# oleg-savchenko/jax_nbody_emulator_with_dj

Measured on AMD Instinct MI355X. Metric: voxels/sec (disp+vel) on 512^3 box, ndiv=4, higher is better.
Workload: dtype f32-equivalent: f16x3 split MFMA (3 f16 MFMAs per product, f32 accumulate)

## Files before the change

jax_nbody_emulator_with_dj_amd/csrc/nbe_engine.cpp:

```cpp

#include "../../include/nbe.h"
#include "nbe_kernels.h"

#include <sched.h>

#include <cmath>
#include <cstdarg>
#include <cstdio>
#include <cstdlib>
#include <cstring>
#include <algorithm>
#include <atomic>
#include <chrono>
#include <condition_variable>
#include <deque>
#include <map>
#include <memory>
#include <mutex>
#include <string>
#include <thread>
#include <vector>

using namespace nbe;

// ... 1261 lines not shown
                                  "up_r2", "conv_r2", "up_r1", "conv_r1", "up_r0", "conv_r00", "conv_r01"};

static int pack_wino(nbe_ctx* c) {
    c->wino_ok = false;
    if (!((c->prec == PREC_F16X3 && (c->vel ? c->gauge_active : true)) || (c->prec == PREC_F16 && c->vel && c->gauge_active))) return 0;
    if (!c->wino_flag) HIPCHK(hipMalloc((void**)&c->wino_flag, 4));
    HIPCHK(hipMemsetAsync(c->wino_flag, 0, 4, c->stream));
    for (auto& kv : c->layers) {
        Layer& L = kv.second;
        if (L.pw.ww && L.kind == 0 && (L.g6 || !c->vel)) launch_pack_h3w(L.wn, L.cout, L.cin, L.pw.cin_pad, L.pw.ctiles, L.pw.ww, c->wino_flag, c->stream, c->prec);
        if (L.pw.ww && L.kind == 1 && (c->vel ? (L.b_sub && c->fuse) : c->novel_fuse)) {
            launch_pack_h3w_skip(L.wn, L.cout, L.cin, L.pw, L.pw.ww, c->wino_flag, c->stream);
            if (c->vel) launch_pack_h3w_skip(c->prec == PREC_F16 ? L.dwn_f : L.dwn, L.cout, L.cin, L.pw, L.pw.ww + L.pw.floats, c->wino_flag, c->stream);
        }
    }
    int bad = 0;
    HIPCHK(hipMemcpyAsync(&bad, c->wino_flag, 4, hipMemcpyDeviceToHost, c->stream));
    HIPCHK(hipStreamSynchronize(c->stream));
    c->wino_ok = bad == 0;
    if (!c->vel) c->fuse = c->novel_fuse && c->wino_ok;
    if (c->prec == PREC_F16) c->fuse = c->fuse && c->wino_ok;
    return 0;
}

static int wire_novel(nbe_ctx* c) {
    c->novel_fuse = false;
    if (c->vel || c->prec != PREC_F16X3) return 0;
    for (const char* b : kBlocks) {
        if (!strncmp(b, "down_", 5) || !strncmp(b, "up_", 3)) continue;
        auto i1 = c->layers.find(std::string(b) + "/conv_1"), is = c->layers.find(std::string(b) + "/skip");
        if (i1 == c->layers.end() || is == c->layers.end()) return fail("internal: block %s", b);
        Layer &L1 = i1->second, &Ls = is->second;
        if (!L1.pw.ww || !Ls.pw.ww || 2 * (Ls.pw.cin_pad / 16) > 16 || L1.pw.ctiles != Ls.pw.ctiles) return 0;
    }
    for (const char* b : kBlocks) {
        if (!strncmp(b, "down_", 5) || !strncmp(b, "up_", 3)) continue;
        Layer &L1 = c->layers[std::string(b) + "/conv_1"], &Ls = c->layers[std::string(b) + "/skip"];
        L1.fskip = &Ls;
        const int nb = L1.pw.ctiles * 32 * L1.pw.ni;
        HIPCHK(hipMalloc((void**)&L1.bias_f, nb * 4));
    }
    c->novel_fuse = true;
    return 0;
}

static int wire_gauge(nbe_ctx* c) {
    const int m = c->mid;
    for (auto& kv : c->layers) {
        Layer& L = kv.second;
        const size_t na = (size_t)roundup(L.cin, 16) + 64, nb = (size_t)L.pw.ctiles * 32 * L.pw.ni + 64;
        HIPCHK(hipMalloc((void**)&L.alpha, na * 4)); HIPCHK(hipMemset(L.alpha, 0, na * 4));
        HIPCHK(hipMalloc((void**)&L.beta, nb * 4)); HIPCHK(hipMemset(L.beta, 0, nb * 4));
    }
    if (!c->gauge_flag) HIPCHK(hipMalloc((void**)&c->gauge_flag, 4));
    auto lay = [&](const char* b, const char* l) -> Layer* {
        auto it = c->layers.find(std::string(b) + "/" + l);
        return it == c->layers.end() ? nullptr : &it->second;
    };
    struct Rule { const char* pb; const char* pl; const char* consumer; int off; };
    const Rule rules[] = {
        {"conv_l00", "conv_1", "conv_l01", 0}, {"conv_l01", "conv_1", "conv_r00", 0}, {"down_l0", "conv_0", "conv_l1", 0},
        {"conv_l1", "conv_1", "conv_r1", 0},   {"down_l1", "conv_0", "conv_l2", 0},   {"conv_l2", "conv_1", "conv_r2", 0},
        {"down_l2", "conv_0", "conv_c", 0},    {"up_r2", "conv_0", "conv_r2", m},     {"up_r1", "conv_0", "conv_r1", m},
        {"up_r0", "conv_0", "conv_r00", m},    {"conv_r00", "conv_1", "conv_r01", 0},
    };
    for (const Rule& r : rules) {
        Layer *P = lay(r.pb, r.pl), *C = lay(r.consumer, "conv_0");
        if (!P || !C || r.off + P->cout > C->cin) return fail("internal: gauge wiring %s/%s -> %s", r.pb, r.pl, r.consumer);
        P->gout = C->alpha + r.off;
    }
    for (const char* b : kBlocks) {
        if (!strncmp(b, "down_", 5) || !strncmp(b, "up_", 3)) continue;
        Layer *L0 = lay(b, "conv_0"), *L1 = lay(b, "conv_1"), *Ls = lay(b, "skip");
        L0->gout = L1->alpha;
        L1->g6 = true;
        if (strcmp(b, "conv_l00")) { L0->g6 = true; Ls->a_in = L0->alpha; }
        if (c->prec == PREC_F16X3 && (!L1->pwn.w || Ls->pwn.dw) &&
            3 * (L1->pw.cin_pad / 16) + Ls->pw.cin_pad / 16 <= NBE_MAX_GROUPS) {
            L1->fskip = Ls; Ls->b_sub = L1->beta;
            const int nb = L1->pw.ctiles * 32 * L1->pw.ni;
            HIPCHK(hipMalloc((void**)&L1->bias_f, nb * 4));
        }
        if (c->prec == PREC_F16 && L1->pw.ww && Ls->pw.ww && Ls->dwn_f && L1->pw.ctiles == Ls->pw.ctiles &&
            2 * (Ls->pw.cin_pad / 32) <= 16) {
            L1->fskip = Ls; Ls->b_sub = L1->beta;
            const int nb = L1->pw.ctiles * 32 * L1->pw.ni;
            HIPCHK(hipMalloc((void**)&L1->bias_f, nb * 4));
        }
    }
    for (auto& kv : c->layers)
        if (kv.second.g6 && 3 * (kv.second.pw.cin_pad / 16) > NBE_MAX_GROUPS) { c->gauge = false; return 0; }
    lay("down_l0", "conv_0")->a_in = lay("conv_r00", "conv_0")->alpha;
    lay("down_l1", "conv_0")->a_in = lay("conv_r1", "conv_0")->alpha;
    lay("down_l2", "conv_0")->a_in = lay("conv_r2", "conv_0")->alpha;
    c->gauge = true;
    return 0;
}

static int wire_gauge_premod(nbe_ctx* c, const nbe_layer_desc* descs, int n) {
    std::map<std::string, std::vector<double>> al, be;
    std::map<std::string, const nbe_layer_desc*> by_name;
    for (int i = 0; i < n; ++i) by_name[std::string(descs[i].block) + "/" + descs[i].layer] = &descs[i];
    for (const char* b : kBlocks) {
        if (!strncmp(b, "down_", 5) || !strncmp(b, "up_", 3)) continue;
        for (const char* l : {"conv_0", "conv_1"}) {
            if (!strcmp(b, "conv_l00") && !strcmp(l, "conv_0")) continue;
            const std::string key = std::string(b) + "/" + l;
            const nbe_layer_desc& d = *by_name[key];
            const int co = d.cout, ci = d.cin, k3 = d.k * d.k * d.k;
            std::vector<double> a(ci, 0.0), bt(co, 0.0);
            double dmax = 0.0;
            for (size_t e = 0; e < (size_t)co * ci * k3; ++e) dmax = std::max(dmax, (double)std::fabs(d.dweight[e]));
            for (int iter = 0; iter < 200; ++iter) {
                double change = 0.0;
                for (int i = 0; i < ci; ++i) {
                    double num = 0.0, den = 0.0;
                    for (int o = 0; o < co; ++o)
                        for (int k = 0; k < k3; ++k) {
                            const double w = d.weight[((size_t)o * ci + i) * k3 + k], dw = d.dweight[((size_t)o * ci + i) * k3 + k];
                            num += w * (dw - w * bt[o]); den += w * w;
                        }
                    const double v = den > 0 ? num / den : 0.0;
                    change = std::max(change, std::fabs(v - a[i])); a[i] = v;
                }
                for (int o = 0; o < co; ++o) {
                    double num = 0.0, den = 0.0;
                    for (int i = 0; i < ci; ++i)
                        for (int k = 0; k < k3; ++k) {
                            const double w = d.weight[((size_t)o * ci + i) * k3 + k], dw = d.dweight[((size_t)o * ci + i) * k3 + k];
                            num += w * (dw - w * a[i]); den += w * w;
                        }
                    const double v = den > 0 ? num / den : 0.0;
                    change = std::max(change, std::fabs(v - bt[o])); bt[o] = v;
                }
                if (change < 1e-13) break;
            }
            double res = 0.0;
            for (int o = 0; o < co; ++o)
                for (int i = 0; i < ci; ++i)
                    for (int k = 0; k < k3; ++k) {
                        const size_t e = ((size_t)o * ci + i) * k3 + k;
                        res = std::max(res, std::fabs((double)d.dweight[e] - (double)d.weight[e] * (a[i] + bt[o])));
                    }
            if (!(res <= 2e-6 * dmax + 1e-30)) return 0;
            const double amin = *std::min_element(a.begin(), a.end()), amax = *std::max_element(a.begin(), a.end());
            const double mid = 0.5 * (amin + amax);
            for (double& v : a) v -= mid;
            for (double& v : bt) v += mid;
            if (amax - mid > 64.0) return 0;
            al[key] = a; be[key] = bt;
        }
    }
    if (wire_gauge(c)) return 1;
    if (!c->gauge) return 0;
    for (auto& kv : c->layers) {
        Layer& L = kv.second;
        auto ia = al.find(kv.first);
        if (ia != al.end()) {
            std::vector<float> fa(ia->second.begin(), ia->second.end()), fb(be[kv.first].begin(), be[kv.first].end());
            HIPCHK(hipMemcpy(L.alpha, fa.data(), fa.size() * 4, hipMemcpyHostToDevice));
            HIPCHK(hipMemcpy(L.beta, fb.data(), fb.size() * 4, hipMemcpyHostToDevice));
        }
    }
    auto fold = [&](const char* b, const char* l, const char* reader, int off) -> int {
        const std::string key = std::string(b) + "/" + l;
        const nbe_layer_desc& d = *by_name[key];
        Layer& L = c->layers[key];
// ... 1325 lines not shown
```

jax_nbody_emulator_with_dj_amd/csrc/nbe_kernels_wino.h:

```cpp

#ifndef NBE_EPI_MAX
#define NBE_EPI_MAX 1
#endif
#ifndef NBE_WINO_ZROW
#define NBE_WINO_ZROW 1
#endif
#ifndef NBE_WINO_ITEMREG
#define NBE_WINO_ITEMREG 1
#endif
#ifndef NBE_WINO_LOU
#define NBE_WINO_LOU (NBE_XF_F32 ? 0 : 1)
#endif
constexpr int NBE_MAX_WSTAGES = 32;
constexpr int NBE_MAX_WSKIP = 16;
constexpr float WINO_WSCALE = 16384.0f;
constexpr float WINO_WSCALE_F16 = 256.0f;

struct WinoSrc { const char* xa; const char* xb; long dxd; const char* w; long psb; float sb; int pad_; };

struct WinoKArgs {
    int H, W, Dv, Hv, Wv, Ho, Wo;
    int nchunk, cout_groups, flags, ntiles, tny, tnx;
    int zblock;
    float* y; float* dy; long out_pstride; int out_g0;
    const float* bias; const float* gout; const float* beta;
    const float* r; const float* dr; long res_pstride;
    float inv_scale;
    int nskip;
    long dws_delta;
    WinoSrc st[NBE_MAX_WSTAGES + NBE_MAX_WSKIP];
};

template <bool SKIP, bool NOVEL, bool F16 = false>
__global__ __launch_bounds__(512, 2) void conv_h3w_kernel(WinoKArgs a) {
    static_assert(!(F16 && NOVEL), "the float16 form has no displacement-only variant");
    typedef HGGeom<false> G;
    constexpr int NW = 8, CT = 64, TAPU = G::TAPU, WGU = G::WG, XBASE = G::XBASE, MT = 4, NT = 2, NTILE = 8;
    constexpr int ZROW = G::LDS_UNITS;
    f32x4* lds = lds_h3;
    const half8* L8 = (const half8*)lds_h3;
    half8* L8w = (half8*)lds_h3;
    const int tid = threadIdx.x;
    const int lane = tid & 63;
    const int wave = __builtin_amdgcn_readfirstlane(tid >> 6);
    const int c = lane & 15, q = lane >> 4, kh = q & 1, ks = q >> 1;

    const int nct = (a.cout_groups + 7) / 8;
    const int vt = xcd_tile(blockIdx.x, a.ntiles * nct);
    const int tile = vt / nct, ct = vt - tile * nct;
    const int npair = a.Dv >> 1;
    int zp, ty, tx;
    {
        const int zb = a.zblock;
        const int full = (npair / zb) * zb;
        const int per_blk = zb * a.tny * a.tnx;
        if (tile < (npair / zb) * per_blk) {
            const int blk = tile / per_blk, r = tile - blk * per_blk;
            const int zi = r % zb, tyx = r / zb;
            zp = blk * zb + zi; ty = tyx / a.tnx; tx = tyx - ty * a.tnx;
        } else {
            const int r = tile - (npair / zb) * per_blk, rem = npair - full;
            const int zi = r % rem, tyx = r / rem;
            zp = full + zi; ty = tyx / a.tnx; tx = tyx - ty * a.tnx;
        }
    }
    const int y0 = ty * (NOVEL ? 2 * HP_ROWS : HP_ROWS), x0 = tx * HP_COLS, z0 = 2 * zp;
    const int nst = 4 * a.nchunk;

    const long to = (((long)z0 * a.H + y0) * a.W + x0) * 16;
    const long wcm = (long)ct * nst * WGU * 16, wcs = (long)ct * a.nskip * TAPU * 16;

    struct Nxt { const char *xa, *xb, *w0; long dxd, psb; float sb; } nx;
    auto set_next = [&](int s) {
        const WinoSrc e = a.st[s];
        nx.xa = e.xa + to; nx.xb = e.xb + to; nx.dxd = e.dxd; nx.psb = e.psb; nx.w0 = e.w + (SKIP && s >= nst ? wcs : wcm); nx.sb = e.sb;
    };
    unsigned lane16 = (unsigned)lane << 4;
    asm volatile("" : "+v"(lane16));
    auto dma_w = [&](int buf, int t) {
        const int n = wave + NW * t;
        unsigned l16 = (unsigned)lane;
        if (NBE_WINO_ZROW && !F16) l16 = lane16;
        else asm volatile("v_lshlrev_b32 %0, 4, %0" : "+v"(l16));
        if (n < G::NWI) dma16s(nx.w0 + (long)n * 1024, l16, lds + buf * WGU + n * 64);
    };
    auto dma_raw = [&](int buf) {
        unsigned l16 = (unsigned)lane;
        asm volatile("v_lshlrev_b32 %0, 4, %0" : "+v"(l16));
        dma16s(nx.w0 + (wave < 4 ? 0 : a.dws_delta) + (long)(wave & 3) * 1024, l16, lds + buf * WGU + wave * 64);
#pragma unroll
        for (int t = 0; t < 6; ++t) {
            const int tensor = t / 3, n = wave + NW * (t % 3), pl = n / 6, k = n - 6 * pl;
            const int u = k * 64 + lane;
            const int uu = u < HP_PL ? u : HP_PL - 1;
            const int row = (uu * 241) >> 13, col = uu - row * HP_RS;
            if (u < HP_PL)
                dma16s(nx.xa + (tensor ? nx.dxd : 0) + (long)pl * nx.psb, (unsigned)(row * a.W + col) * 16u,
                       lds + XBASE + buf * HQ_XB + tensor * HQ_XT + pl * HQ_PP + k * 64);
        }
    };
    constexpr bool ITEMREG = NBE_WINO_ITEMREG && !F16;
    int it_uu[3] = {0, 0, 0};
    unsigned it_go[3] = {0u, 0u, 0u};
    if (ITEMREG) {
#pragma unroll
        for (int j = 0; j < 3; ++j) {
            const int u = ((wave + NW * j) % 6) * 64 + lane;
            it_uu[j] = u < HP_PL ? u : HP_PL - 1;
            const int row = (it_uu[j] * 241) >> 13, col = it_uu[j] - row * HP_RS;
            it_go[j] = (unsigned)(row * a.W + col) * 16u;
        }
#pragma unroll
        for (int j = 0; j < 3; ++j) asm volatile("" : "+v"(it_uu[j]), "+v"(it_go[j]));
    }
    auto item_unit = [&](int j, bool& valid) {
        if (ITEMREG) {
            valid = lane < HP_PL - ((wave + NW * j) % 6) * 64;
            return it_uu[j];
        }
        int l = lane;
        asm volatile("" : "+v"(l));
        const int u = ((wave + NW * j) % 6) * 64 + l;
        valid = u < HP_PL;
        return valid ? u : HP_PL - 1;
    };
    auto item_goff_j = [&](int j) {
        if (ITEMREG) return it_go[j];
        bool v;
        const int uu = item_unit(j, v);
        const int row = (uu * 241) >> 13, col = uu - row * HP_RS;
        return (unsigned)(row * a.W + col) * 16u;
    };
    typedef unsigned int u32x4 __attribute__((ext_vector_type(4)));
    struct Stg { half8 ah, al, bh, bl; float sb; };
    auto st_load = [&](int j, Stg& g) {
        const int n = wave + NW * j;
        const long po = ((n / 12) ? nx.dxd : 0) + (long)(((n % 12) / 6) * 2) * nx.psb;
        const char* pa = nx.xa + po;
        const char* pb = nx.xb + po;
        const unsigned go = item_goff_j(j);
        const __amdgpu_buffer_rsrc_t ra = __builtin_amdgcn_make_buffer_rsrc((void*)pa, 0, 0xffffffffu, 0x00027000);
        const __amdgpu_buffer_rsrc_t rb = __builtin_amdgcn_make_buffer_rsrc((void*)pb, 0, 0xffffffffu, 0x00027000);
        const unsigned pso = (unsigned)nx.psb;
        auto ld = [&](half8& d, __amdgpu_buffer_rsrc_t r, unsigned so) {
            const u32x4 v = __builtin_amdgcn_raw_buffer_load_b128(r, go, so, 0);
            d = __builtin_bit_cast(half8, v);
        };
        ld(g.ah, ra, 0); ld(g.al, ra, pso); ld(g.bh, rb, 0); ld(g.bl, rb, pso);
        g.sb = nx.sb;
    };
#if NBE_XF_F32
    struct Xf { u32x4 HI, LO; float t0, t1; unsigned h; };
    auto xf_step = [&](const Stg& g, Xf& x, int k) {
        const int r = k >> 2, m = k & 3;
        const unsigned AH = __builtin_bit_cast(u32x4, g.ah)[r], AL = __builtin_bit_cast(u32x4, g.al)[r];
        const unsigned BH = __builtin_bit_cast(u32x4, g.bh)[r], BL = __builtin_bit_cast(u32x4, g.bl)[r];
        const float inv = H3_INV, sinv = g.sb * H3_INV, sb = g.sb, k2048 = H3_SCALE;
        if (m == 0) {
            asm("v_fma_mix_f32 %0, %1, %2, %3 op_sel:[0,0,0] op_sel_hi:[1,0,1]" : "=v"(x.t0) : "v"(AL), "s"(inv), "v"(AH));
            asm("v_fma_mix_f32 %0, %1, %2, %0 op_sel:[0,0,0] op_sel_hi:[1,0,0]" : "+v"(x.t0) : "v"(BL), "s"(sinv));
            asm("v_fma_mix_f32 %0, %1, %2, %0 op_sel:[0,0,0] op_sel_hi:[1,0,0]" : "+v"(x.t0) : "v"(BH), "s"(sb));
        } else if (m == 1) {
            asm("v_fma_mix_f32 %0, %1, %2, %3 op_sel:[1,0,1] op_sel_hi:[1,0,1]" : "=v"(x.t1) : "v"(AL), "s"(inv), "v"(AH));
            asm("v_fma_mix_f32 %0, %1, %2, %0 op_sel:[1,0,0] op_sel_hi:[1,0,0]" : "+v"(x.t1) : "v"(BL), "s"(sinv));
            asm("v_fma_mix_f32 %0, %1, %2, %0 op_sel:[1,0,0] op_sel_hi:[1,0,0]" : "+v"(x.t1) : "v"(BH), "s"(sb));
        } else if (m == 2) {
            asm("v_cvt_pk_f16_f32 %0, %1, %2" : "=v"(x.h) : "v"(x.t0), "v"(x.t1));
            asm("v_fma_mix_f32 %0, %1, -1.0, %0 op_sel:[0,0,0] op_sel_hi:[1,0,0]" : "+v"(x.t0) : "v"(x.h));
            asm("v_fma_mix_f32 %0, %1, -1.0, %0 op_sel:[1,0,0] op_sel_hi:[1,0,0]" : "+v"(x.t1) : "v"(x.h));
        } else {
            unsigned l;
            asm("v_fma_mixlo_f16 %0, %1, %2, 0 op_sel_hi:[0,0,0]" : "=v"(l) : "v"(x.t0), "s"(k2048));
            asm("v_fma_mixhi_f16 %0, %1, %2, 0 op_sel_hi:[0,0,0]" : "+v"(l) : "v"(x.t1), "s"(k2048));
            x.HI[r] = x.h; x.LO[r] = l;
        }
    };
#else
    struct Xf { u32x4 HI, LO; unsigned s, bb, e1, e2, l1; };
    auto xf_step = [&](const Stg& g, Xf& x, int k) {
        const int r = k >> 2, m = k & 3;
        const unsigned AH = __builtin_bit_cast(u32x4, g.ah)[r], AL = __builtin_bit_cast(u32x4, g.al)[r];
// ... 130 lines not shown
        NBE_SB; MM8h(DY, wh, dxh, slot0 < 0 ? -1 : slot0 + 4, nb, px, false, hooked, [&](int t) { hook(8 + t); }); NBE_SB;
        after3();
        mid();
#if NBE_WINO_LOU
        NBE_SB; MM8(DY, wh, dxl, -1, nb, px); NBE_SB;
#else
        NBE_SB; MM8(DY, wp, dxl, -1, nb, px); NBE_SB;
#endif
        preXl(); preW();
        NBE_SB; MM8(Y, wl, xh, -1, nb, px); NBE_SB;
        preXh();
        NBE_SB; MM8(DY, wl, dxh, -1, nb, px); NBE_SB;
    };

    constexpr int SH4 = HP_RS + 1, SH5 = HP_RS + 2, SH7 = 2 * HP_RS + 1;
    auto stage = [&](f32x4 (&Y)[NTILE], f32x4 (&DY)[NTILE], int s, auto nxt) {
        constexpr int NXT = decltype(nxt)::value;
        constexpr bool px = NXT == 1;
        const bool pre = px && s + 1 != 2 * a.nchunk;
        if (NXT) set_next(s + 1);
        int par = s & 1;
        asm volatile("" : "+s"(par));
        int nb = 1 - par;
        asm volatile("" : "+s"(nb));
        const int wb = par * WGU, xb = XBASE + par * HQ_XB;
        const int wbn = nb * WGU, xbn = XBASE + nb * HQ_XB;
        Stg g;
        Xf xf;
        auto hk = [&](int k) { xf_step(g, xf, k); };
        auto none = [] {};
        if (NXT == 2) dma_raw(nb);
        if (px) st_load(0, g);
        pair(Y, DY, 0, nb, px, wb, xb + bP1,
             [&] { LB(xl, xb + 2 + bP32 + HQ_PP); }, [&] { LA(wh, wb + 2 * TAPU + aP); }, [&] { LB(xh, xb + 2 + bP32); },
             none, false, nohook, none);
        half8 a1[MT], a2[MT], b1x[NT], b1d[NT];
        const int aS = wb + 4 * TAPU + (2 * kh + (F16 ? ks : 0)) * CT + c;
        const int bS = xb + (2 * kh + ks) * HQ_PP + rowp * HP_RS + c + SH4;
        pair(Y, DY, -1, nb, px, wb + 2 * TAPU, xb + 2 + bP32,
             [&] { LB(b1x, bS); }, [&] { LA(a1, aS); }, [&] { LB(b1d, bS + HQ_XT); }, none,
             px, hk, [&] { if (px) { st_write(0, nb, xf); st_load(1, g); } });
        const half8 zero = {0, 0, 0, 0, 0, 0, 0, 0};
        if (F16) {
            NBE_SB; MM8(Y, a1, b1x, -1, 0, false); NBE_SB;
            LB(xl, xb + SH5 + bP32 + HQ_PP); LB(xh, xb + SH5 + bP32); LA(wh, wb + 5 * TAPU + aP);
            NBE_SB; MM8(DY, a1, b1d, -1, 0, false); NBE_SB;
        } else {
#if NBE_WINO_LOU
        NBE_SB; MM8(Y, a1, b1x, -1, 0, false); NBE_SB;
#else
        {
            const _Float16 m1 = ks ? kInv : (_Float16)1.0f;
#pragma unroll
            for (int mt = 0; mt < MT; ++mt) a1[mt] = a1[mt] * m1;
        }
        NBE_SB; MM8(Y, a1, b1x, -1, 0, false, true); NBE_SB;
#endif
#if NBE_WINO_ZROW
        LA(a2, ks ? ZROW + c : aS + CT);
#else
        LA(a2, aS + CT);
#endif
        LB(xl, xb + SH5 + bP32 + HQ_PP);
        NBE_SB; MM8(DY, a1, b1d, -1, 0, false); NBE_SB;
        LB(xh, xb + SH5 + bP32); LA(wh, wb + 5 * TAPU + aP);
#if NBE_WINO_ZROW
        NBE_SB; MM8(Y, a2, b1x, -1, 0, false); NBE_SB;
#else
#pragma unroll
        for (int mt = 0; mt < MT; ++mt) a2[mt] = ks ? zero : a2[mt];
        NBE_SB; MM8(Y, a2, b1x, -1, 0, false, true); NBE_SB;
#endif
        MM8(DY, a2, b1d, -1, 0, false); NBE_SB;
        }
        pair(Y, DY, -1, nb, px, wb + 5 * TAPU, xb + SH5 + bP32,
             [&] { LB(xl, xb + SH7 + bP1 + HQ_PP); }, [&] { LA(wh, wb + 7 * TAPU + aP); }, [&] { LB(xh, xb + SH7 + bP1); },
             none, px, hk, [&] { if (px) { st_write(1, nb, xf); st_load(2, g); } });
        pair(Y, DY, -1, nb, px, wb + 7 * TAPU, xb + SH7 + bP1,
             [&] { if (pre) LB(xl, xbn + bP1 + HQ_PP); }, [&] { if (pre) LA(wh, wbn + aP); }, [&] { if (pre) LB(xh, xbn + bP1); },
             [&] { asm volatile("s_waitcnt vmcnt(0) lgkmcnt(0)\n\ts_barrier" ::: "memory"); },
             px, hk, [&] { if (px) st_write(2, nb, xf); });
    };

    auto raw_stage = [&](f32x4 (&Y)[NTILE], f32x4 (&DY)[NTILE], int s, bool px) {
        if (px) set_next(s + 1);
        int par = s & 1;
        asm volatile("" : "+s"(par));
        int nb = 1 - par;
        asm volatile("" : "+s"(nb));
        const int wb = par * WGU, xb = XBASE + par * HQ_XB;
        if (px) dma_raw(nb);
        half8 a1[MT], a2[MT], d1[MT], d2[MT], bx[NT], bd[NT];
        const half8 zero = {0, 0, 0, 0, 0, 0, 0, 0};
        const _Float16 m1 = ks ? kInv : (_Float16)1.0f;
        const int aS = wb + (2 * kh) * CT + c;
        const int bS = xb + (2 * kh + ks) * HQ_PP + rowp * HP_RS + c + SH4;
        if (F16) {
            const int aF = wb + (2 * kh + ks) * CT + c;
            LA(a1, aF); LB(bx, bS); LB(bd, bS + HQ_XT); LA(d1, aF + TAPU);
            NBE_SB; MM8(Y, a1, bx, -1, 0, false); NBE_SB;
            MM8(DY, a1, bd, -1, 0, false); NBE_SB;
            MM8(DY, d1, bx, -1, 0, false); NBE_SB;
            asm volatile("s_waitcnt vmcnt(0) lgkmcnt(0)\n\ts_barrier" ::: "memory");
            return;
        }
        LA(a1, aS); LB(bx, bS); LA(a2, aS + CT); LB(bd, bS + HQ_XT);
#pragma unroll
        for (int mt = 0; mt < MT; ++mt) a1[mt] = a1[mt] * m1;
        NBE_SB; MM8(Y, a1, bx, -1, 0, false, true); NBE_SB;
        if (!NOVEL) LA(d1, aS + TAPU);
#pragma unroll
        for (int mt = 0; mt < MT; ++mt) a2[mt] = ks ? zero : a2[mt];
        NBE_SB; MM8(Y, a2, bx, -1, 0, false, true); NBE_SB;
        if (!NOVEL) LA(d2, aS + TAPU + CT);
        if (NOVEL || !(a.flags & F_SKIP_NODX)) {
            NBE_SB; MM8(DY, a1, bd, -1, 0, false); NBE_SB;
            MM8(DY, a2, bd, -1, 0, false); NBE_SB;
        }
        if (!NOVEL) {
#pragma unroll
            for (int mt = 0; mt < MT; ++mt) { d1[mt] = d1[mt] * m1; d2[mt] = ks ? zero : d2[mt]; }
            NBE_SB; MM8(DY, d1, bx, -1, 0, false, true); NBE_SB;
            MM8(DY, d2, bx, -1, 0, false, true); NBE_SB;
        }
        asm volatile("s_waitcnt vmcnt(0) lgkmcnt(0)\n\ts_barrier" ::: "memory");
    };

    {
        if (NBE_WINO_ZROW && !F16 && tid < 64) L8w[ZROW + tid] = half8{0, 0, 0, 0, 0, 0, 0, 0};
        set_next(0);
#pragma unroll
        for (int k = 0; k < G::NWS; ++k) dma_w(0, k);
        {
            Stg g0, g1, g2;
            st_load(0, g0); st_load(1, g1); st_load(2, g2);
            st_store(0, 0, g0); st_store(1, 0, g1); st_store(2, 0, g2);
        }
        asm volatile("s_waitcnt vmcnt(0) lgkmcnt(0)" ::: "memory");
        __syncthreads();
        LA(wh, aP); LB(xl, XBASE + bP1 + HQ_PP); LB(xh, XBASE + bP1);
    }

    auto butterfly = [&] {
            asm volatile("s_nop 15\n\ts_nop 15" ::: "memory");
#pragma unroll
            for (int t = 0; t < NTILE; ++t) {
                f32x4 p, m;
#pragma unroll
                for (int e = 0; e < 4; ++e) { p[e] = acc_read(YA[t][e]); m[e] = acc_read(YB[t][e]); }
                YA[t] = p + m; YB[t] = p - m;
                asm volatile("" : "+a"(YA[t]), "+a"(YB[t]));
                __builtin_amdgcn_sched_barrier(0);
#pragma unroll
                for (int e = 0; e < 4; ++e) { p[e] = acc_read(DA[t][e]); m[e] = acc_read(DB[t][e]); }
                DA[t] = p + m; DB[t] = p - m;
                asm volatile("" : "+a"(DA[t]), "+a"(DB[t]));
                __builtin_amdgcn_sched_barrier(0);
            }
            asm volatile("s_nop 7" ::: "memory");
            LA(wh, aP); LB(xl, XBASE + bP1 + HQ_PP); LB(xh, XBASE + bP1);
    };
    const int npairs = 2 * a.nchunk;
    for (int s2 = 0; s2 + 1 < npairs; ++s2) {
        if (s2 == a.nchunk) butterfly();
        stage(YA, DA, 2 * s2, std::integral_constant<int, 1>());
        stage(YB, DB, 2 * s2 + 1, std::integral_constant<int, 1>());
    }
    if (npairs - 1 == a.nchunk) butterfly();
    stage(YA, DA, 2 * npairs - 2, std::integral_constant<int, 1>());
    stage(YB, DB, 2 * npairs - 1, std::integral_constant<int, SKIP ? 2 : 0>());
    if (SKIP) {
        for (int sc = 0; sc < a.nskip; ++sc) {
            raw_stage(YA, DA, nst + 2 * sc, true);
            raw_stage(YB, DB, nst + 2 * sc + 1, sc + 1 < a.nskip);
        }
    }
#undef NBE_SB
#undef SNAKE
    asm volatile("s_nop 15\n\ts_nop 15" ::: "memory");

    const bool act = a.flags & F_ACT, gauge = !NOVEL && a.gout != nullptr;
    f32x4 bv[MT], be[MT], gv[MT];
    int unit[MT];
    bool uok[MT];
#pragma unroll
    for (int mt = 0; mt < MT; ++mt) {
        unit[mt] = ct * (CT / 8) + 2 * mt + ks;
        uok[mt] = unit[mt] < a.cout_groups;
        if (!uok[mt]) unit[mt] = a.cout_groups - 1;
        bv[mt] = *(const f32x4*)(a.bias + unit[mt] * 8 + 4 * kh);
        be[mt] = f32x4{0.f, 0.f, 0.f, 0.f};
        if (!NOVEL) be[mt] = *(const f32x4*)(a.beta + unit[mt] * 8 + 4 * kh);
        gv[mt] = f32x4{0.f, 0.f, 0.f, 0.f};
        if (!NOVEL && gauge) gv[mt] = *(const f32x4*)(a.gout + unit[mt] * 8 + 4 * kh);
    }
#pragma unroll
    for (int mt = 0; mt < MT; ++mt) asm volatile("" : "+v"(bv[mt]), "+v"(be[mt]), "+v"(gv[mt]));
    long ob_mt[MT];
#pragma unroll
    for (int mt = 0; mt < MT; ++mt) ob_mt[mt] = (long)(a.out_g0 + (F16 ? 1 : 2) * unit[mt]) * a.out_pstride * 16 + 8 * kh;
    const long ol_off = a.out_pstride * 16;
    auto epilogue = [&](f32x4 (&Y)[NTILE], f32x4 (&DY)[NTILE], int z) {
        int o[NT];
        bool ook[NT], ook2[NT];
#pragma unroll
        for (int nt = 0; nt < NT; ++nt) {
            const int yy = y0 + rowp, xx = x0 + 16 * nt + c;
            ook[nt] = yy < a.Hv && xx < a.Wv;
            ook2[nt] = NOVEL && yy + HP_ROWS < a.Hv && xx < a.Wv;
            o[nt] = ook[nt] ? (z * a.Ho + yy) * a.Wo + xx : z * a.Ho * a.Wo;
        }
        half4 r0[F16 ? NTILE : 1], r1[F16 ? NTILE : 1];
        const bool res = F16 && (a.flags & F_RES);
        if (F16 && res) {
#pragma unroll
            for (int t = 0; t < NTILE; ++t) {
                const int mt = t / NT, nt = t % NT;
                const long rb = ((long)unit[mt] * a.res_pstride + (long)o[nt]) * 16 + 8 * kh;
                r0[t] = *(const half4*)((const char*)a.r + rb);
                r1[t] = *(const half4*)((const char*)a.dr + rb);
            }
#pragma unroll
            for (int t = 0; t < NTILE; ++t) asm volatile("" : "+v"(r0[t]), "+v"(r1[t]));
        }
#pragma unroll
        for (int mt = 0; mt < MT; ++mt) {
#pragma unroll
            for (int nt = 0; nt < NT; ++nt) {
                const int t = mt * NT + nt;
                f32x4 v, dv;
                __builtin_amdgcn_sched_barrier(0);
#pragma unroll
                for (int e = 0; e < 4; ++e) {
                    const float yp = acc_read(Y[t][e]) * a.inv_scale;
                    v[e] = yp + bv[mt][e];
                    dv[e] = acc_read(DY[t][e]) * a.inv_scale + be[mt][e] * yp;
                }
                if (F16 && res) {
#pragma unroll
                    for (int e = 0; e < 4; ++e) { v[e] += (float)r0[t][e]; dv[e] += (float)r1[t][e]; }
                }
                if (act) {
#pragma unroll
                    for (int e = 0; e < 4; ++e) {
                        dv[e] = v[e] > 0.f ? dv[e] : 0.01f * dv[e];
                        v[e] = (F16 || !NBE_EPI_MAX) ? (v[e] >= 0.f ? v[e] : 0.01f * v[e]) : __builtin_fmaxf(v[e], 0.01f * v[e]);
                    }
                }
                if (gauge) {
#pragma unroll
                    for (int e = 0; e < 4; ++e) dv[e] += gv[mt][e] * v[e];
                }
                if (F16) {
                    if (uok[mt] && ook[nt]) {
                        const long ob = ob_mt[mt] + (long)o[nt] * 16;
                        half4 h, dh;
#pragma unroll
                        for (int e = 0; e < 4; ++e) { h[e] = (_Float16)v[e]; dh[e] = (_Float16)dv[e]; }
// ... 7 lines not shown
                        dv[e] = acc_read(DY[t][e]) * a.inv_scale + bv[mt][e];
                        if (act) dv[e] = dv[e] >= 0.f ? dv[e] : 0.01f * dv[e];
                    }
                    const long ob = ob_mt[mt] + (long)o[nt] * 16;
                    const long ol = ob + ol_off;
                    const long r8 = (long)HP_ROWS * a.Wo * 16;
                    half4 hi, lo;
                    if (uok[mt] && ook[nt]) {
                        split4(v, hi, lo);
                        *(half4*)((char*)a.y + ob) = hi;
                        *(half4*)((char*)a.y + ol) = lo;
                    }
                    if (uok[mt] && ook2[nt]) {
                        split4(dv, hi, lo);
                        *(half4*)((char*)a.y + ob + r8) = hi;
                        *(half4*)((char*)a.y + ol + r8) = lo;
                    }
                } else
                if (uok[mt] && ook[nt]) {
                    const long ob = ob_mt[mt] + (long)o[nt] * 16;
                    const long ol = ob + ol_off;
                    half4 hi, lo;
                    split4(v, hi, lo);
                    *(half4*)((char*)a.y + ob) = hi;
                    *(half4*)((char*)a.y + ol) = lo;
                    split4(dv, hi, lo);
                    *(half4*)((char*)a.dy + ob) = hi;
                    *(half4*)((char*)a.dy + ol) = lo;
                }
            }
        }
    };
    epilogue(YA, DA, z0);
    epilogue(YB, DB, z0 + 1);
}

__global__ __launch_bounds__(256) void pack_h3w_kernel(const float* __restrict__ w, int cout, int cin, int nchunk, long total,
                                                       _Float16* __restrict__ dst, int* __restrict__ flag, int f16) {
    const long idx = (long)blockIdx.x * blockDim.x + threadIdx.x;
    if (idx >= total) return;
    long r = idx;
    const int j = (int)(r % 8); r /= 8;
    const int co = (int)(r % 64); r /= 64;
    const int u = (int)(r % 4); r /= 4;
    const int tap = (int)(r % 9); r /= 9;
    const int stage = (int)(r % (4 * nchunk)); r /= 4 * nchunk;
    const int ct = (int)r;
    const int chunk = stage >> 2, xi = stage & 3;
    const int h = u >> 1, part = u & 1;
    const int ci = f16 ? chunk * 32 + 8 * u + j : chunk * 16 + 8 * h + j, oc = ct * 64 + co;
    float v = 0.f;
    if (oc < cout && ci < cin) {
        const float* p = w + (((size_t)oc * cin + ci) * 3) * 9 + tap;
        const float w0 = p[0], w1 = p[9], w2 = p[18];
        v = xi == 0 ? w0 : xi == 1 ? 0.5f * (w0 + w1 + w2) : xi == 2 ? 0.5f * (w0 - w1 + w2) : -w2;
    }
    v *= f16 ? WINO_WSCALE_F16 : WINO_WSCALE;
    if (!(fabsf(v) <= 60000.f)) { atomicOr(flag, 1); v = 0.f; }
    const _Float16 hi = (_Float16)v;
    dst[idx] = (part == 0 || f16) ? hi : (_Float16)(v - (float)hi);
}

void launch_pack_h3w(const float* w_oidhw, int cout, int cin, int cin_pad, int ctiles, float* dst, int* flag, hipStream_t s, int prec) {
    const bool f16 = prec == PREC_F16;
    const int nchunk = cin_pad / (f16 ? 32 : 16);
    const long total = (long)ctiles * 4 * nchunk * 9 * 4 * 64 * 8;
    hipLaunchKernelGGL(pack_h3w_kernel, dim3((unsigned)((total + 255) / 256)), dim3(256), 0, s, w_oidhw, cout, cin, nchunk, total,
                       (_Float16*)dst, flag, f16 ? 1 : 0);
}

static int launch_h3w(const ConvKArgs& ka_in, const float* ww, const float* wws, long wws_set_floats, int ctiles, hipStream_t s,
                      bool novel = false, bool f16 = false) {
    typedef HGGeom<false> G;
    constexpr size_t smem = (size_t)(G::LDS_UNITS + 64) * 16;
    static_assert(smem <= 160 * 1024, "LDS budget of one CU");
    ConvKArgs ka = ka_in;
    if (f16) {
        if (novel || (ka.nchunk & 1) || (ka.csplit < ka.nchunk && (ka.csplit & 1))) return 1;
        if (ka.nskip > 0 && ((ka.nskip & 1) || (ka.s_csplit < ka.nskip && (ka.s_csplit & 1)) || (ka.flags & F_SKIP_NODX))) return 1;
        ka.nchunk /= 2; if (ka.csplit < (1 << 29)) ka.csplit /= 2;
        ka.nskip /= 2; if (ka.s_csplit < (1 << 29)) ka.s_csplit /= 2;
    }
    if (!ww || (!f16 && (ka.flags & F_RES)) || (ka.Dv & 1) || 4 * ka.nchunk > NBE_MAX_WSTAGES || (!novel && !ka.beta)) return 1;
    if (ka.nskip > 0 && (!wws || 2 * ka.nskip > NBE_MAX_WSKIP)) return 1;
    if (ctiles != (ka.cout_groups + 7) / 8) return 1;
    if (std::max(ka.in_pstride, ka.csplit < ka.nchunk ? ka.in2_pstride : 0L) * 16 + 16L * (HP_ROWS + 2) * ka.W >= (1L << 32) - (1L << 20)) return 1;
    WinoKArgs wa;
    wa.H = ka.H; wa.W = ka.W; wa.Dv = ka.Dv; wa.Hv = ka.Hv; wa.Wv = ka.Wv; wa.Ho = ka.Ho; wa.Wo = ka.Wo;
    wa.nchunk = ka.nchunk; wa.cout_groups = ka.cout_groups; wa.flags = ka.flags;
    const int trows = novel ? 2 * HP_ROWS : HP_ROWS;
    wa.tny = (ka.Hv + trows - 1) / trows;
    wa.tnx = (ka.Wv + HP_COLS - 1) / HP_COLS;
    wa.ntiles = (ka.Dv / 2) * wa.tny * wa.tnx;
    wa.y = ka.y; wa.dy = ka.dy; wa.out_pstride = ka.out_pstride; wa.out_g0 = ka.out_g0;
    wa.bias = ka.bias; wa.gout = novel ? nullptr : ka.gout; wa.beta = novel ? nullptr : ka.beta;
    const long rows8 = (long)HP_ROWS * ka.W * 16;
    wa.inv_scale = 1.0f / (f16 ? WINO_WSCALE_F16 : WINO_WSCALE);
    wa.r = ka.r; wa.dr = ka.dr; wa.res_pstride = ka.res_pstride;
    wa.zblock = std::min(8, ka.Dv / 2);
    wa.nskip = ka.nskip; wa.dws_delta = wws_set_floats * 4;
    static const int XI[2][2] = {{1, 2}, {0, 3}};
    static const int PA[4] = {0, 1, 2, 1}, PB[4] = {2, 2, 1, 3};
    static const float SB[4] = {-1.f, 1.f, -1.f, -1.f};
    const long plane = (long)ka.H * ka.W * 16;
    for (int ph = 0; ph < 2; ++ph)
        for (int chunk = 0; chunk < ka.nchunk; ++chunk)
            for (int ab = 0; ab < 2; ++ab) {
                const int xi = XI[ph][ab];
                const bool second = chunk >= ka.csplit;
                const long ps = second ? ka.in2_pstride : ka.in_pstride;
                const char* x = (const char*)(second ? ka.x2 : ka.x);
                const char* dx = (const char*)(second ? ka.dx2 : ka.dx);
                const long off = (long)(second ? chunk - ka.csplit : chunk) * 4 * ps * 16;
                WinoSrc& e = wa.st[(ph * ka.nchunk + chunk) * 2 + ab];
                e.xa = x + off + PA[xi] * plane; e.xb = x + off + PB[xi] * plane; e.dxd = novel ? rows8 : dx - x;
                e.w = (const char*)ww + (long)(chunk * 4 + xi) * G::WG * 16; e.psb = ps * 16; e.sb = SB[xi]; e.pad_ = 0;
            }
    for (int sc = 0; sc < ka.nskip; ++sc)
        for (int ab = 0; ab < 2; ++ab) {
            const bool second = sc >= ka.s_csplit;
            const long ps = second ? ka.s2_pstride : ka.s_pstride;
            const char* x = (const char*)(second ? ka.xs2 : ka.xs);
            const char* dx = (const char*)(second ? ka.dxs2 : ka.dxs);
            const long off = (long)(second ? sc - ka.s_csplit : sc) * 4 * ps * 16 + ab * plane;
            WinoSrc& e = wa.st[4 * ka.nchunk + 2 * sc + ab];
            e.xa = x + off; e.xb = e.xa; e.dxd = novel ? rows8 : dx - x; e.w = (const char*)wws + (long)sc * G::TAPU * 16; e.psb = ps * 16; e.sb = 0.f; e.pad_ = 0;
        }
    const bool skip = ka.nskip > 0;
    if (novel) wa.dws_delta = 0;
    auto kern = f16 ? (skip ? conv_h3w_kernel<true, false, true> : conv_h3w_kernel<false, false, true>)
              : novel ? (skip ? conv_h3w_kernel<true, true> : conv_h3w_kernel<false, true>)
              : (skip ? conv_h3w_kernel<true, false> : conv_h3w_kernel<false, false>);
    ensure_lds_limit((const void*)kern, smem);
    dim3 grid(wa.ntiles * ctiles, 1, 1), block(512, 1, 1);
    hipLaunchKernelGGL(kern, grid, block, smem, s, wa);
    return 0;
}
```

Baseline: 97.06 million.

## Merge paired raw skip stages into one chunk stage sharing weights per barrier

The fused skip (raw 1x1) phase in the Winograd h3w kernel used to run two stages per skip chunk, one for each of the A and B output planes, each with its own DMA and barrier. It now loads both planes' inputs plus one weight set into a single LDS slot with a new compact layout, and issues the MFMAs for both accumulators from shared A-operand registers. This halves the number of barriers and weight loads in the skip tail, and on the f32 path reuses the zero-row trick instead of masking in registers. The skip stage table and the limits are halved to match, which adds new LDS layout constraints guarded by a static_assert.

```diff
diff --git a/jax_nbody_emulator_with_dj_amd/csrc/nbe_engine.cpp b/jax_nbody_emulator_with_dj_amd/csrc/nbe_engine.cpp
--- a/jax_nbody_emulator_with_dj_amd/csrc/nbe_engine.cpp
+++ b/jax_nbody_emulator_with_dj_amd/csrc/nbe_engine.cpp
@@ -1367,7 +1367,7 @@
             HIPCHK(hipMalloc((void**)&L1->bias_f, nb * 4));
         }
         if (c->prec == PREC_F16 && L1->pw.ww && Ls->pw.ww && Ls->dwn_f && L1->pw.ctiles == Ls->pw.ctiles &&
-            2 * (Ls->pw.cin_pad / 32) <= 16) {
+            Ls->pw.cin_pad / 32 <= 8) {
             L1->fskip = Ls; Ls->b_sub = L1->beta;
             const int nb = L1->pw.ctiles * 32 * L1->pw.ni;
             HIPCHK(hipMalloc((void**)&L1->bias_f, nb * 4));
diff --git a/jax_nbody_emulator_with_dj_amd/csrc/nbe_kernels_wino.h b/jax_nbody_emulator_with_dj_amd/csrc/nbe_kernels_wino.h
--- a/jax_nbody_emulator_with_dj_amd/csrc/nbe_kernels_wino.h
+++ b/jax_nbody_emulator_with_dj_amd/csrc/nbe_kernels_wino.h
@@ -12,7 +12,7 @@
 #define NBE_WINO_LOU (NBE_XF_F32 ? 0 : 1)
 #endif
 constexpr int NBE_MAX_WSTAGES = 32;
-constexpr int NBE_MAX_WSKIP = 16;
+constexpr int NBE_MAX_WSKIP = 8;
 constexpr float WINO_WSCALE = 16384.0f;
 constexpr float WINO_WSCALE_F16 = 256.0f;
 
@@ -84,19 +84,21 @@
         else asm volatile("v_lshlrev_b32 %0, 4, %0" : "+v"(l16));
         if (n < G::NWI) dma16s(nx.w0 + (long)n * 1024, l16, lds + buf * WGU + n * 64);
     };
-    auto dma_raw = [&](int buf) {
-        unsigned l16 = (unsigned)lane;
-        asm volatile("v_lshlrev_b32 %0, 4, %0" : "+v"(l16));
-        dma16s(nx.w0 + (wave < 4 ? 0 : a.dws_delta) + (long)(wave & 3) * 1024, l16, lds + buf * WGU + wave * 64);
-#pragma unroll
-        for (int t = 0; t < 6; ++t) {
-            const int tensor = t / 3, n = wave + NW * (t % 3), pl = n / 6, k = n - 6 * pl;
-            const int u = k * 64 + lane;
-            const int uu = u < HP_PL ? u : HP_PL - 1;
-            const int row = (uu * 241) >> 13, col = uu - row * HP_RS;
-            if (u < HP_PL)
-                dma16s(nx.xa + (tensor ? nx.dxd : 0) + (long)pl * nx.psb, (unsigned)(row * a.W + col) * 16u,
-                       lds + XBASE + buf * HQ_XB + tensor * HQ_XT + pl * HQ_PP + k * 64);
+    constexpr int RAW_SP = HP_ROWS * HP_COLS, RAW_XT = 4 * RAW_SP, RAW_W = 2 * RAW_XT;
+    static_assert(RAW_W + 2 * TAPU <= HQ_XB && RAW_W <= WGU, "a chunk of the raw phase fits one slot");
+    auto dma_raw = [&](int slot) {
+        int l = lane;
+        asm volatile("" : "+v"(l));
+        dma16s(nx.w0 + (wave < 4 ? 0 : a.dws_delta) + (long)(wave & 3) * 1024, (unsigned)l << 4,
+               lds + XBASE + slot * HQ_XB + RAW_W + wave * 64);
+        const unsigned lo = (unsigned)((l >> 5) * a.W + (l & 31)) * 16u;
+        const int k = wave & 3, h = wave >> 2;
+        const long ro = ((long)(2 * k + 1) * a.W + 1) * 16;
+#pragma unroll
+        for (int t = 0; t < 8; ++t) {
+            const int ab = t >> 2, tensor = (t >> 1) & 1, pl = h + 2 * (t & 1);
+            dma16s((ab ? nx.xb : nx.xa) + (tensor ? nx.dxd : 0) + (long)pl * nx.psb + ro, lo,
+                   lds + (ab ? slot * WGU : XBASE + slot * HQ_XB) + tensor * RAW_XT + pl * RAW_SP + k * 64);
         }
     };
     constexpr bool ITEMREG = NBE_WINO_ITEMREG && !F16;
@@ -393,46 +395,68 @@
              px, hk, [&] { if (px) st_write(2, nb, xf); });
     };
 
-    auto raw_stage = [&](f32x4 (&Y)[NTILE], f32x4 (&DY)[NTILE], int s, bool px) {
-        if (px) set_next(s + 1);
-        int par = s & 1;
-        asm volatile("" : "+s"(par));
-        int nb = 1 - par;
-        asm volatile("" : "+s"(nb));
-        const int wb = par * WGU, xb = XBASE + par * HQ_XB;
-        if (px) dma_raw(nb);
-        half8 a1[MT], a2[MT], d1[MT], d2[MT], bx[NT], bd[NT];
-        const half8 zero = {0, 0, 0, 0, 0, 0, 0, 0};
-        const _Float16 m1 = ks ? kInv : (_Float16)1.0f;
-        const int aS = wb + (2 * kh) * CT + c;
-        const int bS = xb + (2 * kh + ks) * HQ_PP + rowp * HP_RS + c + SH4;
+    auto raw_chunk = [&](int sc, bool px) {
+        if (px) set_next(nst + sc + 1);
+        int k = sc & 1;
+        asm volatile("" : "+s"(k));
+        int nk = 1 - k;
+        asm volatile("" : "+s"(nk));
+        if (px) dma_raw(nk);
+        const int xs = XBASE + k * HQ_XB, ws = xs + RAW_W;
+        const int pb = (2 * kh + ks) * RAW_SP + rowp * HP_COLS + c;
+        const int bA = xs + pb, bB = k * WGU + pb;
+        half8 a1[MT], a2[MT], d1[MT], d2[MT], bx[NT], bd[NT], bx2[NT];
         if (F16) {
-            const int aF = wb + (2 * kh + ks) * CT + c;
-            LA(a1, aF); LB(bx, bS); LB(bd, bS + HQ_XT); LA(d1, aF + TAPU);
-            NBE_SB; MM8(Y, a1, bx, -1, 0, false); NBE_SB;
-            MM8(DY, a1, bd, -1, 0, false); NBE_SB;
-            MM8(DY, d1, bx, -1, 0, false); NBE_SB;
+            const int aF = ws + (2 * kh + ks) * CT + c;
+            LA(a1, aF); LB(bx, bA); LB(bd, bA + RAW_XT); LA(d1, aF + TAPU);
+            NBE_SB; MM8(YA, a1, bx, -1, 0, false); NBE_SB;
+            LB(bx2, bB);
+            MM8(DA, a1, bd, -1, 0, false); NBE_SB;
+            LB(bd, bB + RAW_XT);
+            MM8(DA, d1, bx, -1, 0, false); NBE_SB;
+            MM8(YB, a1, bx2, -1, 0, false); NBE_SB;
+            MM8(DB, a1, bd, -1, 0, false); NBE_SB;
+            MM8(DB, d1, bx2, -1, 0, false); NBE_SB;
             asm volatile("s_waitcnt vmcnt(0) lgkmcnt(0)\n\ts_barrier" ::: "memory");
             return;
         }
-        LA(a1, aS); LB(bx, bS); LA(a2, aS + CT); LB(bd, bS + HQ_XT);
+        const _Float16 m1 = ks ? kInv : (_Float16)1.0f;
+        const int aS = ws + (2 * kh) * CT + c;
+        const bool zrow = NBE_WINO_ZROW;
+        const half8 zero = {0, 0, 0, 0, 0, 0, 0, 0};
+        LA(a1, aS); LB(bx, bA); LA(a2, zrow && ks ? ZROW + c : aS + CT); LB(bd, bA + RAW_XT);
 #pragma unroll
         for (int mt = 0; mt < MT; ++mt) a1[mt] = a1[mt] * m1;
-        NBE_SB; MM8(Y, a1, bx, -1, 0, false, true); NBE_SB;
+        NBE_SB; MM8(YA, a1, bx, -1, 0, false, true); NBE_SB;
         if (!NOVEL) LA(d1, aS + TAPU);
-#pragma unroll
-        for (int mt = 0; mt < MT; ++mt) a2[mt] = ks ? zero : a2[mt];
-        NBE_SB; MM8(Y, a2, bx, -1, 0, false, true); NBE_SB;
-        if (!NOVEL) LA(d2, aS + TAPU + CT);
-        if (NOVEL || !(a.flags & F_SKIP_NODX)) {
-            NBE_SB; MM8(DY, a1, bd, -1, 0, false); NBE_SB;
-            MM8(DY, a2, bd, -1, 0, false); NBE_SB;
+        LB(bx2, bB);
+        if (!zrow) {
+#pragma unroll
+            for (int mt = 0; mt < MT; ++mt) a2[mt] = ks ? zero : a2[mt];
+        }
+        NBE_SB; MM8(YA, a2, bx, -1, 0, false, !zrow); NBE_SB;
+        if (!NOVEL) LA(d2, zrow && ks ? ZROW + c : aS + TAPU + CT);
+        const bool dxp = NOVEL || !(a.flags & F_SKIP_NODX);
+        if (dxp) {
+            NBE_SB; MM8(DA, a1, bd, -1, 0, false); NBE_SB;
+            MM8(DA, a2, bd, -1, 0, false); NBE_SB;
+            LB(bd, bB + RAW_XT);
         }
         if (!NOVEL) {
 #pragma unroll
-            for (int mt = 0; mt < MT; ++mt) { d1[mt] = d1[mt] * m1; d2[mt] = ks ? zero : d2[mt]; }
-            NBE_SB; MM8(DY, d1, bx, -1, 0, false, true); NBE_SB;
-            MM8(DY, d2, bx, -1, 0, false, true); NBE_SB;
+            for (int mt = 0; mt < MT; ++mt) { d1[mt] = d1[mt] * m1; if (!zrow) d2[mt] = ks ? zero : d2[mt]; }
+            NBE_SB; MM8(DA, d1, bx, -1, 0, false, true); NBE_SB;
+            MM8(DA, d2, bx, -1, 0, false, !zrow); NBE_SB;
+        }
+        NBE_SB; MM8(YB, a1, bx2, -1, 0, false); NBE_SB;
+        MM8(YB, a2, bx2, -1, 0, false); NBE_SB;
+        if (dxp) {
+            MM8(DB, a1, bd, -1, 0, false); NBE_SB;
+            MM8(DB, a2, bd, -1, 0, false); NBE_SB;
+        }
+        if (!NOVEL) {
+            MM8(DB, d1, bx2, -1, 0, false); NBE_SB;
+            MM8(DB, d2, bx2, -1, 0, false); NBE_SB;
         }
         asm volatile("s_waitcnt vmcnt(0) lgkmcnt(0)\n\ts_barrier" ::: "memory");
     };
@@ -481,10 +505,7 @@
     stage(YA, DA, 2 * npairs - 2, std::integral_constant<int, 1>());
     stage(YB, DB, 2 * npairs - 1, std::integral_constant<int, SKIP ? 2 : 0>());
     if (SKIP) {
-        for (int sc = 0; sc < a.nskip; ++sc) {
-            raw_stage(YA, DA, nst + 2 * sc, true);
-            raw_stage(YB, DB, nst + 2 * sc + 1, sc + 1 < a.nskip);
-        }
+        for (int sc = 0; sc < a.nskip; ++sc) raw_chunk(sc, sc + 1 < a.nskip);
     }
 #undef NBE_SB
 #undef SNAKE
@@ -658,7 +679,7 @@
         ka.nskip /= 2; if (ka.s_csplit < (1 << 29)) ka.s_csplit /= 2;
     }
     if (!ww || (!f16 && (ka.flags & F_RES)) || (ka.Dv & 1) || 4 * ka.nchunk > NBE_MAX_WSTAGES || (!novel && !ka.beta)) return 1;
-    if (ka.nskip > 0 && (!wws || 2 * ka.nskip > NBE_MAX_WSKIP)) return 1;
+    if (ka.nskip > 0 && (!wws || ka.nskip > NBE_MAX_WSKIP)) return 1;
     if (ctiles != (ka.cout_groups + 7) / 8) return 1;
     if (std::max(ka.in_pstride, ka.csplit < ka.nchunk ? ka.in2_pstride : 0L) * 16 + 16L * (HP_ROWS + 2) * ka.W >= (1L << 32) - (1L << 20)) return 1;
     WinoKArgs wa;
@@ -692,16 +713,15 @@
                 e.xa = x + off + PA[xi] * plane; e.xb = x + off + PB[xi] * plane; e.dxd = novel ? rows8 : dx - x;
                 e.w = (const char*)ww + (long)(chunk * 4 + xi) * G::WG * 16; e.psb = ps * 16; e.sb = SB[xi]; e.pad_ = 0;
             }
-    for (int sc = 0; sc < ka.nskip; ++sc)
-        for (int ab = 0; ab < 2; ++ab) {
-            const bool second = sc >= ka.s_csplit;
-            const long ps = second ? ka.s2_pstride : ka.s_pstride;
-            const char* x = (const char*)(second ? ka.xs2 : ka.xs);
-            const char* dx = (const char*)(second ? ka.dxs2 : ka.dxs);
-            const long off = (long)(second ? sc - ka.s_csplit : sc) * 4 * ps * 16 + ab * plane;
-            WinoSrc& e = wa.st[4 * ka.nchunk + 2 * sc + ab];
-            e.xa = x + off; e.xb = e.xa; e.dxd = novel ? rows8 : dx - x; e.w = (const char*)wws + (long)sc * G::TAPU * 16; e.psb = ps * 16; e.sb = 0.f; e.pad_ = 0;
-        }
+    for (int sc = 0; sc < ka.nskip; ++sc) {
+        const bool second = sc >= ka.s_csplit;
+        const long ps = second ? ka.s2_pstride : ka.s_pstride;
+        const char* x = (const char*)(second ? ka.xs2 : ka.xs);
+        const char* dx = (const char*)(second ? ka.dxs2 : ka.dxs);
+        const long off = (long)(second ? sc - ka.s_csplit : sc) * 4 * ps * 16;
+        WinoSrc& e = wa.st[4 * ka.nchunk + sc];
+        e.xa = x + off; e.xb = e.xa + plane; e.dxd = novel ? rows8 : dx - x; e.w = (const char*)wws + (long)sc * G::TAPU * 16; e.psb = ps * 16; e.sb = 0.f; e.pad_ = 0;
+    }
     const bool skip = ka.nskip > 0;
     if (novel) wa.dws_delta = 0;
     auto kern = f16 ? (skip ? conv_h3w_kernel<true, false, true> : conv_h3w_kernel<false, false, true>)
```

Result: no change. 97.99 million, median of 6 (+1.0%).
